# Ewenwan/ORB_SLAM2_SSD_Semantic

Hardware: AMD Instinct MI355X
Metric: ORB extract+match frames/sec on 640x480 TUM RGB-D; bit-exact kp/desc (higher is better)
Workload: dtype u8

## Files before the change

### orb_slam2_ssd_semantic_amd/csrc/orbfe_match.hip

```cpp
#include <stddef.h>
#include <algorithm>
#include <new>

#include <vector>

#include "orbfe_common.h"
#include "orbfe_kernels.h"
#include "orbfe_matcher.h"
#include "orbfe_match_dev.h"

#define BM_WAVES 4
#define BM_QUERIES(Q) (BM_WAVES * (Q) * 32)
#define BM_NEG (-(1 << 30))
#define BM_MAX_NT (1 << 22)

typedef int bm_v4i __attribute__((ext_vector_type(4)));
typedef int bm_v16i __attribute__((ext_vector_type(16)));

__device__ __forceinline__ uint2 bm_expand_byte(uint32_t v, uint32_t mag)
{
    uint32_t lo = 0, hi = 0;
#pragma unroll
    for (int b = 0; b < 4; ++b) {
        lo |= (((v >> b) & 1u) ? mag : (0x100u - mag)) << (8 * b);
        hi |= (((v >> (4 + b)) & 1u) ? mag : (0x100u - mag)) << (8 * b);
    }
    return make_uint2(lo, hi);
}

template <int BM_Q>
__global__ __launch_bounds__(BM_WAVES * 64, 2) void k_match_bf(const uint8_t *__restrict__ q_base,
                                                               const uint8_t *__restrict__ t_base,
                                                               const int32_t *__restrict__ n_arr,
                                                               const int32_t *__restrict__ tn_arr,
                                                               const int32_t *__restrict__ qframe,
                                                               const int32_t *__restrict__ tframe, int cap, int nq_s,
                                                               int nt_s, float nnratio, int th,
                                                               int32_t *__restrict__ match, int32_t *__restrict__ best_o,
                                                               int32_t *__restrict__ second_o)
{
    __shared__ uint2 s_tabq[256], s_tabt[256];
    __shared__ __attribute__((aligned(16))) uint8_t s_tile[2][32 * 256];
    const int pair = blockIdx.y;
    const uint8_t *q = q_base, *t = t_base;
    int nq = nq_s, nt = nt_s;
    int64_t out0 = 0;
    if (n_arr) {
        const int qf = qframe[pair], tf = tframe[pair];
        q = q_base + (int64_t)qf * cap * 32;
        t = t_base + (int64_t)tf * cap * 32;
        nq = min(n_arr[qf], cap);
        nt = min(tn_arr[tf], cap);
        out0 = (int64_t)pair * cap;
    }
    const int tid = threadIdx.x, lane = tid & 63;
    const int wid = __builtin_amdgcn_readfirstlane(tid >> 6);
    constexpr int BM_QW = BM_QUERIES(BM_Q);
    const int q0 = blockIdx.x * BM_QW;
    const int nslots = n_arr ? cap : nq;
    if (q0 >= nslots) return;
    if (q0 >= nq) {
        for (int i = q0 + tid; i < min(q0 + BM_QW, nslots); i += BM_WAVES * 64) {
            match[out0 + i] = -1;
            if (best_o) best_o[out0 + i] = 256;
            if (second_o) second_o[out0 + i] = 256;
        }
        return;
    }
    s_tabq[tid] = bm_expand_byte((uint32_t)tid, 1u);
    s_tabt[tid] = bm_expand_byte((uint32_t)tid, 64u);
    __syncthreads();

    const int c = lane & 31, h = lane >> 5;
    bm_v4i B[BM_Q][8];
#pragma unroll
    for (int u = 0; u < BM_Q; ++u) {
        const int qi = q0 + (wid * BM_Q + u) * 32 + c;
        const uint4 raw = *(const uint4 *)(q + (int64_t)min(qi, nq - 1) * 32 + h * 16);
        const uint32_t rw[4] = {raw.x, raw.y, raw.z, raw.w};
#pragma unroll
        for (int sstep = 0; sstep < 8; ++sstep) {
            const uint32_t b0 = (rw[sstep >> 1] >> (16 * (sstep & 1))) & 0xFFu;
            const uint32_t b1 = (rw[sstep >> 1] >> (16 * (sstep & 1) + 8)) & 0xFFu;
            const uint2 e0 = s_tabq[b0], e1 = s_tabq[b1];
            B[u][sstep] = bm_v4i{(int)e0.x, (int)e0.y, (int)e1.x, (int)e1.y};
        }
    }
    int kb[BM_Q], ks[BM_Q], bi[BM_Q];
#pragma unroll
    for (int u = 0; u < BM_Q; ++u) {
        kb[u] = ks[u] = BM_NEG;
        bi[u] = -1;
    }
    if (nt > 0) {
        const int sr = tid & 31, sw = tid >> 5;
        const uint32_t *t32 = (const uint32_t *)t;
        auto stage_load = [&](int T) -> uint32_t { return t32[(uint32_t)(min(T + sr, nt - 1) * 8 + sw)]; };
        auto stage_store = [&](uint32_t dw, int buf) {
#pragma unroll
            for (int i = 0; i < 4; ++i) {
                const int beta = 4 * sw + i, hh = beta >> 4, bp = beta & 15;
                const int off = (((bp >> 1) * 2 + hh) * 32 + sr) * 16 + (bp & 1) * 8;
                *(uint2 *)(s_tile[buf] + off) = s_tabt[(dw >> (8 * i)) & 0xFFu];
            }
        };
        auto load_a = [&](bm_v4i (&A)[8], int buf) {
#pragma unroll
            for (int sstep = 0; sstep < 8; ++sstep)
                A[sstep] = *(const bm_v4i *)(s_tile[buf] + ((sstep * 2 + h) * 32 + c) * 16);
        };
        bm_v16i cfull;
#pragma unroll
        for (int reg = 0; reg < 16; ++reg) cfull[reg] = 32 - ((reg & 3) + 8 * (reg >> 2) + 4 * h);
        auto chain = [&](const bm_v4i (&A)[8], const bm_v4i (&Bu)[8]) -> bm_v16i {
            bm_v16i acc = cfull;
#pragma unroll
            for (int sstep = 0; sstep < 8; ++sstep) acc = __builtin_amdgcn_mfma_i32_32x32x32_i8(A[sstep], Bu[sstep], acc, 0, 0, 0);
            return acc;
        };
        auto interleave = [&]() {
#pragma unroll
            for (int g = 0; g < 8; ++g) {
                __builtin_amdgcn_sched_group_barrier(0x008, 1, 0);
                __builtin_amdgcn_sched_group_barrier(0x002, 5, 0);
            }
            __builtin_amdgcn_sched_barrier(0);
        };
        auto rank = [&](const bm_v16i &acc, int u, int T, bool mask_tail) {
            int hi[8], lo[8];
#pragma unroll
            for (int p = 0; p < 8; ++p) {
                int k0 = acc[2 * p], k1 = acc[2 * p + 1];
                if (mask_tail) {
                    if (T + ((2 * p) & 3) + 8 * ((2 * p) >> 2) + 4 * h >= nt) k0 = BM_NEG;
                    if (T + ((2 * p + 1) & 3) + 8 * ((2 * p + 1) >> 2) + 4 * h >= nt) k1 = BM_NEG;
                }
                hi[p] = max(k0, k1);
                lo[p] = min(k0, k1);
            }
#pragma unroll
            for (int w = 4; w >= 1; w >>= 1)
#pragma unroll
                for (int p = 0; p < w; ++p) {
                    const int h2 = max(hi[p], hi[p + w]);
                    lo[p] = max(min(hi[p], hi[p + w]), max(lo[p], lo[p + w]));
                    hi[p] = h2;
                }
            const int bprev = kb[u] | 127, sprev = ks[u] | 127;
            const int b = max(bprev, hi[0]);
            const int s2 = max(min(bprev, hi[0]), max(sprev, lo[0]));
            if (b != bprev) bi[u] = T + 32 - (b & 127);
            kb[u] = b;
            ks[u] = s2;
        };

        stage_store(stage_load(0), 0);
        uint32_t g1 = stage_load(32);
        __syncthreads();
        bm_v4i A[8];
        load_a(A, 0);
        bm_v16i acc = chain(A, B[0]);
        int buf = 0, T = 0;
        for (; T + 32 < nt; T += 32) {
            const uint32_t g2 = stage_load(T + 64);
            stage_store(g1, buf ^ 1);
            g1 = g2;
#pragma unroll
            for (int u = 0; u < BM_Q; ++u) {
                bm_v16i nacc;
                if (u + 1 < BM_Q) {
                    nacc = chain(A, B[u + 1]);
                } else {
                    __syncthreads();
                    buf ^= 1;
                    load_a(A, buf);
                    nacc = chain(A, B[0]);
                }
                rank(acc, u, T, false);
                interleave();
                acc = nacc;
            }
        }
#pragma unroll
        for (int u = 0; u < BM_Q; ++u) {
            bm_v16i nacc = acc;
            if (u + 1 < BM_Q) nacc = chain(A, B[u + 1]);
            rank(acc, u, T, true);
            acc = nacc;
        }
    }
#pragma unroll
    for (int u = 0; u < BM_Q; ++u) {
        const int ob = __shfl_xor(kb[u], 32, 64), os = __shfl_xor(ks[u], 32, 64), oi = __shfl_xor(bi[u], 32, 64);
        const int mb = kb[u] >> 7, mo = ob >> 7;
        const bool take_o = mo > mb || (mo == mb && oi >= 0 && (bi[u] < 0 || oi < bi[u]));
        const int m1 = take_o ? mo : mb, idx = take_o ? oi : bi[u];
        const int m2 = max(min(mb, mo), max(ks[u] >> 7, os >> 7));
        const int qi = q0 + (wid * BM_Q + u) * 32 + c;
        if (h == 0 && qi < nslots) {
            const int best = idx >= 0 ? 128 - m1 : 256;
            const int second = m2 > (BM_NEG >> 8) ? 128 - m2 : 256;
            const bool valid = qi < nq;
            int m = -1;
            if (valid && idx >= 0 && best < 256 && best <= th && (float)best < __fmul_rn(nnratio, (float)second)) m = idx;
            match[out0 + qi] = m;
            if (best_o) best_o[out0 + qi] = valid ? best : 256;
            if (second_o) second_o[out0 + qi] = valid ? second : 256;
        }
    }
}

#define BP_TILE 128
__global__ __launch_bounds__(256) void k_match_popc(const uint8_t *__restrict__ q_base, const uint8_t *__restrict__ t_base,
                                                    const int32_t *__restrict__ n_arr, const int32_t *__restrict__ tn_arr,
                                                    const int32_t *__restrict__ qframe,
                                                    const int32_t *__restrict__ tframe, int cap, int nq_s, int nt_s,
                                                    float nnratio, int th, int32_t *__restrict__ match,
                                                    int32_t *__restrict__ best_o, int32_t *__restrict__ second_o)
{
    __shared__ uint4 s_t[BP_TILE][2];
    const int pair = blockIdx.y;
    const uint8_t *q = q_base, *t = t_base;
    int nq = nq_s, nt = nt_s;
    int64_t out0 = 0;
    if (n_arr) {
        const int qf = qframe[pair], tf = tframe[pair];
        q = q_base + (int64_t)qf * cap * 32;
        t = t_base + (int64_t)tf * cap * 32;
        nq = min(n_arr[qf], cap);
        nt = min(tn_arr[tf], cap);
        out0 = (int64_t)pair * cap;
    }
    const int tid = threadIdx.x;
    const int qi = blockIdx.x * 256 + tid;
    const int nslots = n_arr ? cap : nq;
    if ((int)blockIdx.x * 256 >= nslots) return;
    uint32_t qw[8];
    {
        const uint4 *pq = (const uint4 *)(q + (int64_t)min(qi, max(nq - 1, 0)) * 32);
        const uint4 a = nq > 0 ? pq[0] : make_uint4(0, 0, 0, 0), b = nq > 0 ? pq[1] : make_uint4(0, 0, 0, 0);
        qw[0] = a.x; qw[1] = a.y; qw[2] = a.z; qw[3] = a.w; qw[4] = b.x; qw[5] = b.y; qw[6] = b.z; qw[7] = b.w;
    }
    uint32_t k1 = 0xFFFFFFFFu, k2 = 0xFFFFFFFFu;
    for (int T = 0; T < nt; T += BP_TILE) {
        __syncthreads();
        {
            const int r = tid >> 1, hf = tid & 1;
            s_t[r][hf] = ((const uint4 *)(t + (int64_t)min(T + r, nt - 1) * 32))[hf];
        }
        __syncthreads();
        const int rows = min(BP_TILE, nt - T);
        for (int r = 0; r < rows; ++r) {
            const uint4 a = s_t[r][0], b = s_t[r][1];
            uint32_t d = __popc(qw[0] ^ a.x);
            d += __popc(qw[1] ^ a.y);
            d += __popc(qw[2] ^ a.z);
            d += __popc(qw[3] ^ a.w);
            d += __popc(qw[4] ^ b.x);
            d += __popc(qw[5] ^ b.y);
            d += __popc(qw[6] ^ b.z);
            d += __popc(qw[7] ^ b.w);
            const uint32_t k = (d << 22) | (uint32_t)(T + r);
            k2 = min(k2, max(k1, k));
            k1 = min(k1, k);
        }
    }
    if (qi < nslots) {
        const bool valid = qi < nq;
        const int best = k1 != 0xFFFFFFFFu ? (int)(k1 >> 22) : 256;
        const int second = k2 != 0xFFFFFFFFu ? (int)(k2 >> 22) : 256;
        const int idx = k1 != 0xFFFFFFFFu ? (int)(k1 & 0x3FFFFFu) : -1;
        int m = -1;
        if (valid && idx >= 0 && best < 256 && best <= th && (float)best < __fmul_rn(nnratio, (float)second)) m = idx;
        match[out0 + qi] = m;
        if (best_o) best_o[out0 + qi] = valid ? best : 256;
        if (second_o) second_o[out0 + qi] = valid ? second : 256;
    }
}

__global__ __launch_bounds__(256) void k_rot_prune(int32_t *__restrict__ match, const float *__restrict__ a_ang,
                                                   const float *__restrict__ b_ang, int ang_stride,
                                                   const int32_t *__restrict__ n_arr,
                                                   const int32_t *__restrict__ aframe,
                                                   const int32_t *__restrict__ bframe, int cap, int n_s,
                                                   int check_ori, int32_t *__restrict__ nmatches)
{
    __shared__ int s_hist[ORBFE_HISTO_LENGTH];
    __shared__ int s_keep[3];
    __shared__ int s_count;
    const int pair = blockIdx.x, tid = threadIdx.x;
    int n = n_s;
    int32_t *mt = match;
    const float *aa = a_ang, *ba = b_ang;
    if (n_arr) {
        const int af = aframe[pair], bf = bframe[pair];
        n = min(n_arr[af], cap);
        mt = match + (int64_t)pair * cap;
        aa = a_ang + (int64_t)af * cap * ang_stride;
        ba = b_ang + (int64_t)bf * cap * ang_stride;
    }
    if (tid < ORBFE_HISTO_LENGTH) s_hist[tid] = 0;
    if (tid == 0) s_count = 0;
    __syncthreads();
    if (check_ori) {
        for (int i = tid; i < n; i += 256) {
            const int j = mt[i];
            if (j >= 0) atomicAdd(&s_hist[rot_bin(aa[(int64_t)i * ang_stride], ba[(int64_t)j * ang_stride])], 1);
        }
        __syncthreads();
        if (tid == 0) {
            int max1 = 0, max2 = 0, max3 = 0, i1 = -1, i2 = -1, i3 = -1;
            for (int i = 0; i < ORBFE_HISTO_LENGTH; ++i) {
                const int s = s_hist[i];
                if (s > max1) {
                    max3 = max2; max2 = max1; max1 = s;
                    i3 = i2; i2 = i1; i1 = i;
                } else if (s > max2) {
                    max3 = max2; max2 = s;
                    i3 = i2; i2 = i;
                } else if (s > max3) {
                    max3 = s; i3 = i;
                }
            }
            if ((float)max2 < __fmul_rn(0.1f, (float)max1)) { i2 = -1; i3 = -1; }
            else if ((float)max3 < __fmul_rn(0.1f, (float)max1)) { i3 = -1; }
            s_keep[0] = i1; s_keep[1] = i2; s_keep[2] = i3;
        }
        __syncthreads();
    }
    int local = 0;
    for (int i = tid; i < n; i += 256) {
        const int j = mt[i];
        if (j < 0) continue;
        if (check_ori) {
            const int bin = rot_bin(aa[(int64_t)i * ang_stride], ba[(int64_t)j * ang_stride]);
            if (bin != s_keep[0] && bin != s_keep[1] && bin != s_keep[2]) {
                mt[i] = -1;
                continue;
            }
        }
        ++local;
    }
    atomicAdd(&s_count, local);
    __syncthreads();
    if (tid == 0) nmatches[pair] = s_count;
}

__global__ __launch_bounds__(256) void k_hamming_csr(const uint8_t *__restrict__ q, int nq,
                                                     const uint8_t *__restrict__ t, const uint32_t *__restrict__ off,
                                                     const uint32_t *__restrict__ cand, int32_t *__restrict__ best_idx,
                                                     int32_t *__restrict__ best, int32_t *__restrict__ second,
                                                     int32_t *__restrict__ second_idx)
{
    const int i = blockIdx.x * 256 + threadIdx.x;
    if (i >= nq) return;
    Desc8 dq;
    const uint32_t *p = (const uint32_t *)(q + (int64_t)i * 32);
#pragma unroll
    for (int k = 0; k < 8; ++k) dq.w[k] = p[k];
    int b1 = 256, b2 = 256, bi = -1, si = -1;
    for (uint32_t j = off[i]; j < off[i + 1]; ++j) {
        const uint32_t c = cand[j];
        const int d = hamming8(dq, (const uint32_t *)(t + (int64_t)c * 32));
        if (d < b1) { b2 = b1; si = bi; b1 = d; bi = (int)c; }
        else if (d < b2) { b2 = d; si = (int)c; }
    }
    best_idx[i] = bi;
    best[i] = b1;
    second[i] = b2;
    if (second_idx) second_idx[i] = si;
}

__global__ __launch_bounds__(256) void k_hamming_csr_all(const uint8_t *__restrict__ q, int nq, const uint8_t *__restrict__ t,
                                                         const uint32_t *__restrict__ off, const uint32_t *__restrict__ cand,
                                                         uint16_t *__restrict__ dist)
{
    const int i = blockIdx.x * 4 + (threadIdx.x >> 6);
    if (i >= nq) return;
    const int lane = threadIdx.x & 63;
    Desc8 dq;
    const uint32_t *p = (const uint32_t *)(q + (int64_t)i * 32);
#pragma unroll
    for (int k = 0; k < 8; ++k) dq.w[k] = p[k];
    const uint32_t e = off[i + 1];
    for (uint32_t j = off[i] + (uint32_t)lane; j < e; j += 64u)
        dist[j] = (uint16_t)hamming8(dq, (const uint32_t *)(t + (int64_t)cand[j] * 32));
}

extern "C" int32_t orbfe_hamming(const uint8_t a[32], const uint8_t b[32])
{
    int d = 0;
    for (int i = 0; i < 8; ++i) {
        uint32_t x, y;
        memcpy(&x, a + 4 * i, 4);
        memcpy(&y, b + 4 * i, 4);
        d += __builtin_popcount(x ^ y);
    }
    return d;
}

static orbfe_status matcher_create_impl(int32_t device, hipStream_t borrowed, bool borrow, orbfe_matcher **out);
extern "C" orbfe_status orbfe_matcher_create(int32_t device, orbfe_matcher **out) { return matcher_create_impl(device, nullptr, false, out); }
orbfe_status orbfe_internal_matcher_create_on_stream(int32_t device, void *st, orbfe_matcher **out)
{
    return matcher_create_impl(device, (hipStream_t)st, true, out);
}

static orbfe_status matcher_create_impl(int32_t device, hipStream_t borrowed, bool borrow, orbfe_matcher **out)
{
    if (!out) return ORBFE_ERR_ARG;
    *out = nullptr;
    const orbfe_status rs = orb_resolve_device(&device);
    if (rs != ORBFE_OK) return rs;
    orbfe_matcher *m = new (std::nothrow) orbfe_matcher();
    if (!m) return ORBFE_ERR_NOMEM;
    m->device = device;
    DeviceGuard g(device);
    m->own_stream = !borrow;
    if (borrow) m->stream = borrowed;
    if ((!borrow && hipStreamCreateWithFlags(&m->stream, hipStreamNonBlocking) != hipSuccess) ||
        hipEventCreateWithFlags(&m->ev_scratch, hipEventDisableTiming) != hipSuccess) {
        orbfe_set_error("hipStreamCreate / hipEventCreate failed");
        if (m->stream && m->own_stream) (void)hipStreamDestroy(m->stream);
        delete m;
        return ORBFE_ERR_HIP;
    }
    *out = m;
    return ORBFE_OK;
}

extern "C" void *orbfe_matcher_get_stream(orbfe_matcher *m) { return m ? (void *)m->stream : nullptr; }

extern "C" orbfe_status orbfe_matcher_set_bf_kernel(orbfe_matcher *m, int32_t kernel)
{
    if (!m || kernel < 0 || kernel > 1) return ORBFE_ERR_ARG;
    m->bf_kernel = kernel;
    return ORBFE_OK;
}

extern "C" orbfe_status orbfe_internal_matcher_set_bf_tiles(orbfe_matcher *m, int32_t tiles)
{
    if (!m || !orb_match_tiles_ok(tiles)) return ORBFE_ERR_ARG;
    m->bf_tiles = tiles;
    return ORBFE_OK;
}

extern "C" orbfe_status orbfe_matcher_set_projection_kernel(orbfe_matcher *m, int32_t kernel)
{
    if (!m || kernel < 0 || kernel > 1) return ORBFE_ERR_ARG;
    m->proj_fused = kernel == 0;
    return ORBFE_OK;
}

extern "C" void orbfe_matcher_destroy(orbfe_matcher *m)
{
    if (!m) return;
    DeviceGuard g(m->device);
    if (m->stream) (void)hipStreamSynchronize(m->stream);
    if (m->scratch_used) (void)hipEventSynchronize(m->ev_scratch);
    for (auto &b : m->b) b.release();
    m->proj_done.release();
    m->pin_in.release();
    m->pin_out.release();
    if (m->ev_scratch) (void)hipEventDestroy(m->ev_scratch);
    if (m->stream && m->own_stream) (void)hipStreamDestroy(m->stream);
    delete m;
}

template <typename... Args>
static void launch_match_bf(int tiles, int nslots, int npairs, hipStream_t st, Args... args)
{
    const dim3 block(BM_WAVES * 64);
    auto grid = [&](int qw) { return dim3((nslots + qw - 1) / qw, npairs); };
    if (tiles == 1) hipLaunchKernelGGL(k_match_bf<1>, grid(BM_QUERIES(1)), block, 0, st, args...);
    else if (tiles == 2) hipLaunchKernelGGL(k_match_bf<2>, grid(BM_QUERIES(2)), block, 0, st, args...);
    else hipLaunchKernelGGL(k_match_bf<4>, grid(BM_QUERIES(4)), block, 0, st, args...);
}

static orbfe_status launch_bf(int kernel, int tiles, const uint8_t *d_q, int nq, const uint8_t *d_t, int nt, const float *d_qa,
                              const float *d_ta, int ang_stride, float nnratio, int th, int check_ori,
                              int32_t *d_match, int32_t *d_best, int32_t *d_second, int32_t *d_nm, hipStream_t st)
{
    if (nq > 0) {
        if (kernel == 1)
            hipLaunchKernelGGL(k_match_popc, dim3((nq + 255) / 256, 1), dim3(256), 0, st, d_q, d_t, (const int32_t *)nullptr,
                               (const int32_t *)nullptr, (const int32_t *)nullptr, (const int32_t *)nullptr, 0, nq, nt, nnratio, th,
                               d_match, d_best, d_second);
        else
            launch_match_bf(tiles, nq, 1, st, d_q, d_t, (const int32_t *)nullptr, (const int32_t *)nullptr, (const int32_t *)nullptr,
                            (const int32_t *)nullptr, 0, nq, nt, nnratio, th, d_match, d_best, d_second);
        ORBFE_HIP(hipGetLastError());
    }
    const int ori = (check_ori && d_qa && d_ta) ? 1 : 0;
    hipLaunchKernelGGL(k_rot_prune, dim3(1), dim3(256), 0, st, d_match, d_qa, d_ta, ang_stride,
                       (const int32_t *)nullptr, (const int32_t *)nullptr, (const int32_t *)nullptr, 0, nq, ori, d_nm);
    ORBFE_HIP(hipGetLastError());
    return ORBFE_OK;
}

extern "C" orbfe_status orbfe_match_bf_device(orbfe_matcher *m, const uint8_t *d_q, int32_t nq, const uint8_t *d_t,
                                              int32_t nt, const float *d_q_angle, const float *d_t_angle,
                                              float nnratio, int32_t th, int32_t check_ori, int32_t *d_match_q2t,
                                              int32_t *d_best, int32_t *d_second, int32_t *d_nmatches, void *stream)
{
    if (!m || nq < 0 || nt < 0 || nt > BM_MAX_NT || !d_match_q2t || !d_nmatches || (nq > 0 && !d_q) || (nt > 0 && !d_t)) {
        orbfe_set_error("bad argument to orbfe_match_bf_device (train set limited to %d descriptors)", BM_MAX_NT);
        return ORBFE_ERR_ARG;
    }
    DeviceGuard g(m->device);
    return launch_bf(m->bf_kernel, m->bf_tiles, d_q, nq, d_t, nt, d_q_angle, d_t_angle, 1, nnratio, th, check_ori, d_match_q2t, d_best, d_second,
                     d_nmatches, (hipStream_t)stream);
}

extern "C" orbfe_status orbfe_match_bf(orbfe_matcher *m, const uint8_t *q, int32_t nq, const uint8_t *t, int32_t nt,
                                       const float *q_angle, const float *t_angle, float nnratio, int32_t th,
                                       int32_t check_ori, int32_t *match_q2t, int32_t *best, int32_t *second,
                                       int32_t *nmatches)
{
    if (!m || nq < 0 || nt < 0 || nt > BM_MAX_NT || (nq > 0 && (!q || !match_q2t)) || (nt > 0 && !t)) {
        orbfe_set_error("bad argument to orbfe_match_bf (train set limited to %d descriptors)", BM_MAX_NT);
        return ORBFE_ERR_ARG;
    }
    if (nq == 0) {
        if (nmatches) *nmatches = 0;
        return ORBFE_OK;
    }
    DeviceGuard g(m->device);
    hipStream_t st = m->stream;
    ORBFE_HIP(scratch_acquire(m, st));
    const bool ori = check_ori && q_angle && t_angle;
    ORBFE_HIP(m->b[0].ensure((size_t)nq * 32));
    ORBFE_HIP(m->b[1].ensure((size_t)nt * 32));
    ORBFE_HIP(m->b[2].ensure((size_t)nq * 4));
    ORBFE_HIP(m->b[3].ensure((size_t)nt * 4));
    ORBFE_HIP(m->b[4].ensure((size_t)nq * 4));
    ORBFE_HIP(m->b[5].ensure((size_t)nq * 4));
    ORBFE_HIP(m->b[6].ensure((size_t)nq * 4));
    ORBFE_HIP(m->b[7].ensure(4));
    ORBFE_HIP(hipMemcpyAsync(m->b[0].p, q, (size_t)nq * 32, hipMemcpyHostToDevice, st));
    if (nt > 0) ORBFE_HIP(hipMemcpyAsync(m->b[1].p, t, (size_t)nt * 32, hipMemcpyHostToDevice, st));
    if (ori) {
        ORBFE_HIP(hipMemcpyAsync(m->b[2].p, q_angle, (size_t)nq * 4, hipMemcpyHostToDevice, st));
        if (nt > 0) ORBFE_HIP(hipMemcpyAsync(m->b[3].p, t_angle, (size_t)nt * 4, hipMemcpyHostToDevice, st));
    }
    orbfe_status s = launch_bf(m->bf_kernel, m->bf_tiles, m->b[0].as<const uint8_t>(), nq, m->b[1].as<const uint8_t>(), nt,
                               ori ? m->b[2].as<const float>() : nullptr, ori ? m->b[3].as<const float>() : nullptr, 1,
                               nnratio, th, ori ? 1 : 0, m->b[4].as<int32_t>(), m->b[5].as<int32_t>(),
                               m->b[6].as<int32_t>(), m->b[7].as<int32_t>(), st);
    if (s != ORBFE_OK) return s;
    int32_t nm = 0;
    ORBFE_HIP(hipMemcpyAsync(match_q2t, m->b[4].p, (size_t)nq * 4, hipMemcpyDeviceToHost, st));
    if (best) ORBFE_HIP(hipMemcpyAsync(best, m->b[5].p, (size_t)nq * 4, hipMemcpyDeviceToHost, st));
    if (second) ORBFE_HIP(hipMemcpyAsync(second, m->b[6].p, (size_t)nq * 4, hipMemcpyDeviceToHost, st));
    ORBFE_HIP(hipMemcpyAsync(&nm, m->b[7].p, 4, hipMemcpyDeviceToHost, st));
    ORBFE_HIP(hipStreamSynchronize(st));
    if (nmatches) *nmatches = nm;
    return ORBFE_OK;
}

extern "C" orbfe_status orbfe_match_bf_blocks_device(orbfe_matcher *m, const orbfe_keypoint *d_qkps, const uint8_t *d_qdesc,
                                                     const int32_t *d_qn, const orbfe_keypoint *d_tkps, const uint8_t *d_tdesc,
                                                     const int32_t *d_tn, int32_t cap, const int32_t *d_qframe,
                                                     const int32_t *d_tframe, int32_t npairs, float nnratio, int32_t th,
                                                     int32_t check_ori, int32_t *d_match_q2t, int32_t *d_nmatches, void *stream)
{
    return orbfe_internal_match_bf_blocks_tiles(m, d_qkps, d_qdesc, d_qn, d_tkps, d_tdesc, d_tn, cap, d_qframe, d_tframe, npairs, nnratio, th,
                                                check_ori, d_match_q2t, d_nmatches, m ? m->bf_tiles : 0, stream);
}

orbfe_status orbfe_internal_match_bf_blocks_tiles(orbfe_matcher *m, const orbfe_keypoint *d_qkps, const uint8_t *d_qdesc,
                                                  const int32_t *d_qn, const orbfe_keypoint *d_tkps, const uint8_t *d_tdesc,
                                                  const int32_t *d_tn, int32_t cap, const int32_t *d_qframe, const int32_t *d_tframe,
                                                  int32_t npairs, float nnratio, int32_t th, int32_t check_ori, int32_t *d_match_q2t,
                                                  int32_t *d_nmatches, int32_t tiles, void *stream)
{
    if (!m || !d_qkps || !d_qdesc || !d_qn || !d_tkps || !d_tdesc || !d_tn || !d_qframe || !d_tframe || !d_match_q2t ||
        !d_nmatches || cap < 1 || cap > BM_MAX_NT || npairs < 0 || !orb_match_tiles_ok(tiles)) {
        orbfe_set_error("bad argument to orbfe_match_bf_blocks_device / _frames_device (cap 1..%d)", BM_MAX_NT);
        return ORBFE_ERR_ARG;
    }
    if (npairs == 0) return ORBFE_OK;
    DeviceGuard g(m->device);
    hipStream_t st = (hipStream_t)stream;
    if (m->bf_kernel == 1)
        hipLaunchKernelGGL(k_match_popc, dim3((cap + 255) / 256, npairs), dim3(256), 0, st, d_qdesc, d_tdesc, d_qn, d_tn, d_qframe,
                           d_tframe, cap, 0, 0, nnratio, th, d_match_q2t, (int32_t *)nullptr, (int32_t *)nullptr);
    else
        launch_match_bf(tiles, cap, npairs, st, d_qdesc, d_tdesc, d_qn, d_tn, d_qframe, d_tframe, cap, 0, 0, nnratio, th, d_match_q2t,
                        (int32_t *)nullptr, (int32_t *)nullptr);
    ORBFE_HIP(hipGetLastError());
    hipLaunchKernelGGL(k_rot_prune, dim3(npairs), dim3(256), 0, st, d_match_q2t, &d_qkps->angle, &d_tkps->angle, 7, d_qn, d_qframe,
                       d_tframe, cap, 0, check_ori ? 1 : 0, d_nmatches);
    ORBFE_HIP(hipGetLastError());
    return ORBFE_OK;
}

extern "C" orbfe_status orbfe_match_bf_frames_device(orbfe_matcher *m, const orbfe_keypoint *d_kps,
                                                     const uint8_t *d_desc, const int32_t *d_n, int32_t cap,
                                                     const int32_t *d_qframe, const int32_t *d_tframe, int32_t npairs,
                                                     float nnratio, int32_t th, int32_t check_ori,
                                                     int32_t *d_match_q2t, int32_t *d_nmatches, void *stream)
{
    return orbfe_match_bf_blocks_device(m, d_kps, d_desc, d_n, d_kps, d_desc, d_n, cap, d_qframe, d_tframe, npairs, nnratio, th,
                                        check_ori, d_match_q2t, d_nmatches, stream);
}

extern "C" orbfe_status orbfe_hamming_csr_ex(orbfe_matcher *m, const uint8_t *q, int32_t nq, const uint8_t *t, int32_t nt,
                                             const uint32_t *off, const uint32_t *cand, int32_t *best_idx, int32_t *best,
                                             int32_t *second, int32_t *second_idx)
{
    if (!m || nq < 0 || nt < 0 || (nq > 0 && (!q || !off || !best_idx || !best || !second))) {
        orbfe_set_error("bad argument to orbfe_hamming_csr");
        return ORBFE_ERR_ARG;
    }
    if (nq == 0) return ORBFE_OK;
    const size_t nc = off[nq];
    for (int i = 0; i < nq; ++i)
        if (off[i + 1] < off[i]) { orbfe_set_error("CSR offsets must not decrease"); return ORBFE_ERR_ARG; }
    for (size_t k = 0; k < nc; ++k)
        if (cand[k] >= (uint32_t)nt) { orbfe_set_error("candidate index out of range"); return ORBFE_ERR_ARG; }
    DeviceGuard g(m->device);
    hipStream_t st = m->stream;
    ORBFE_HIP(scratch_acquire(m, st));
    ORBFE_HIP(m->b[0].ensure((size_t)nq * 32));
    ORBFE_HIP(m->b[1].ensure((size_t)nt * 32));
    ORBFE_HIP(m->b[2].ensure((size_t)(nq + 1) * 4));
    ORBFE_HIP(m->b[3].ensure(nc * 4));
    ORBFE_HIP(m->b[4].ensure((size_t)nq * 4));
    ORBFE_HIP(m->b[5].ensure((size_t)nq * 4));
    ORBFE_HIP(m->b[6].ensure((size_t)nq * 4));
    ORBFE_HIP(m->b[7].ensure((size_t)nq * 4));
    ORBFE_HIP(hipMemcpyAsync(m->b[0].p, q, (size_t)nq * 32, hipMemcpyHostToDevice, st));
    if (nt > 0) ORBFE_HIP(hipMemcpyAsync(m->b[1].p, t, (size_t)nt * 32, hipMemcpyHostToDevice, st));
    ORBFE_HIP(hipMemcpyAsync(m->b[2].p, off, (size_t)(nq + 1) * 4, hipMemcpyHostToDevice, st));
    if (nc > 0) ORBFE_HIP(hipMemcpyAsync(m->b[3].p, cand, nc * 4, hipMemcpyHostToDevice, st));
    hipLaunchKernelGGL(k_hamming_csr, dim3((nq + 255) / 256), dim3(256), 0, st, m->b[0].as<const uint8_t>(), nq,
                       m->b[1].as<const uint8_t>(), m->b[2].as<const uint32_t>(), m->b[3].as<const uint32_t>(),
                       m->b[4].as<int32_t>(), m->b[5].as<int32_t>(), m->b[6].as<int32_t>(), m->b[7].as<int32_t>());
    ORBFE_HIP(hipGetLastError());
    if (second_idx) ORBFE_HIP(hipMemcpyAsync(second_idx, m->b[7].p, (size_t)nq * 4, hipMemcpyDeviceToHost, st));
    ORBFE_HIP(hipMemcpyAsync(best_idx, m->b[4].p, (size_t)nq * 4, hipMemcpyDeviceToHost, st));
    ORBFE_HIP(hipMemcpyAsync(best, m->b[5].p, (size_t)nq * 4, hipMemcpyDeviceToHost, st));
    ORBFE_HIP(hipMemcpyAsync(second, m->b[6].p, (size_t)nq * 4, hipMemcpyDeviceToHost, st));
    ORBFE_HIP(hipStreamSynchronize(st));
    return ORBFE_OK;
}

extern "C" orbfe_status orbfe_hamming_csr_all(orbfe_matcher *m, const uint8_t *q, int32_t nq, const uint8_t *t, int32_t nt,
                                              const uint32_t *off, const uint32_t *cand, uint16_t *dist)
{
    if (!m || nq < 0 || nt < 0 || (nq > 0 && (!q || !off))) {
        orbfe_set_error("bad argument to orbfe_hamming_csr_all");
        return ORBFE_ERR_ARG;
    }
    if (nq == 0) return ORBFE_OK;
    const size_t nc = off[nq];
    for (int i = 0; i < nq; ++i)
        if (off[i + 1] < off[i]) { orbfe_set_error("CSR offsets must not decrease"); return ORBFE_ERR_ARG; }
    if (nc == 0) return ORBFE_OK;
    if (!cand || !dist || !t) { orbfe_set_error("bad argument to orbfe_hamming_csr_all"); return ORBFE_ERR_ARG; }
    for (size_t k = 0; k < nc; ++k)
        if (cand[k] >= (uint32_t)nt) { orbfe_set_error("candidate index out of range"); return ORBFE_ERR_ARG; }
    DeviceGuard g(m->device);
    hipStream_t st = m->stream;
    ORBFE_HIP(scratch_acquire(m, st));
    ORBFE_HIP(m->b[0].ensure((size_t)nq * 32));
    ORBFE_HIP(m->b[1].ensure((size_t)nt * 32));
    ORBFE_HIP(m->b[2].ensure((size_t)(nq + 1) * 4));
    ORBFE_HIP(m->b[3].ensure(nc * 4));
    ORBFE_HIP(m->b[4].ensure(nc * 2));
    ORBFE_HIP(hipMemcpyAsync(m->b[0].p, q, (size_t)nq * 32, hipMemcpyHostToDevice, st));
    ORBFE_HIP(hipMemcpyAsync(m->b[1].p, t, (size_t)nt * 32, hipMemcpyHostToDevice, st));
    ORBFE_HIP(hipMemcpyAsync(m->b[2].p, off, (size_t)(nq + 1) * 4, hipMemcpyHostToDevice, st));
    ORBFE_HIP(hipMemcpyAsync(m->b[3].p, cand, nc * 4, hipMemcpyHostToDevice, st));
    hipLaunchKernelGGL(k_hamming_csr_all, dim3((nq + 3) / 4), dim3(256), 0, st, m->b[0].as<const uint8_t>(), nq,
                       m->b[1].as<const uint8_t>(), m->b[2].as<const uint32_t>(), m->b[3].as<const uint32_t>(), m->b[4].as<uint16_t>());
    ORBFE_HIP(hipGetLastError());
    ORBFE_HIP(hipMemcpyAsync(dist, m->b[4].p, nc * 2, hipMemcpyDeviceToHost, st));
    ORBFE_HIP(hipStreamSynchronize(st));
    return ORBFE_OK;
}

extern "C" orbfe_status orbfe_hamming_csr(orbfe_matcher *m, const uint8_t *q, int32_t nq, const uint8_t *t, int32_t nt,
                                          const uint32_t *off, const uint32_t *cand, int32_t *best_idx, int32_t *best,
                                          int32_t *second)
{
    return orbfe_hamming_csr_ex(m, q, nq, t, nt, off, cand, best_idx, best, second, nullptr);
}

extern "C" orbfe_status orbfe_hamming_csr_device(orbfe_matcher *m, const uint8_t *d_q, int32_t nq, const uint8_t *d_t,
                                                 const uint32_t *d_off, const uint32_t *d_cand, int32_t *d_best_idx,
                                                 int32_t *d_best, int32_t *d_second, int32_t *d_second_idx, void *stream)
{
    if (!m || nq < 0 || (nq > 0 && (!d_q || !d_t || !d_off || !d_cand || !d_best_idx || !d_best || !d_second))) {
        orbfe_set_error("bad argument to orbfe_hamming_csr_device");
        return ORBFE_ERR_ARG;
    }
    if (nq == 0) return ORBFE_OK;
    DeviceGuard g(m->device);
    hipLaunchKernelGGL(k_hamming_csr, dim3((nq + 255) / 256), dim3(256), 0, (hipStream_t)stream, d_q, nq, d_t, d_off, d_cand,
                       d_best_idx, d_best, d_second, d_second_idx);
    ORBFE_HIP(hipGetLastError());
    return ORBFE_OK;
}
```

### orb_slam2_ssd_semantic_amd/csrc/orbfe_match_dev.h

```cpp
#pragma once

#include "orbfe_common.h"

#define GRID_NC (ORBFE_GRID_COLS * ORBFE_GRID_ROWS)

struct Desc8 {
    uint32_t w[8];
};

__device__ __forceinline__ int hamming8(const Desc8 &a, const uint32_t *__restrict__ b)
{
    int d = 0;
#pragma unroll
    for (int i = 0; i < 8; ++i) d += __popc(a.w[i] ^ b[i]);
    return d;
}

struct Best2 {
    int best, second, idx;
};

__device__ __forceinline__ Best2 merge_best2(const Best2 &lo, const Best2 &hi)
{
    Best2 r;
    if (hi.best < lo.best) {
        r.best = hi.best;
        r.idx = hi.idx;
        r.second = min(lo.best, hi.second);
    } else {
        r.best = lo.best;
        r.idx = lo.idx;
        r.second = min(lo.second, hi.best);
    }
    return r;
}

__device__ __forceinline__ int rot_bin(float a1, float a2)
{
    const float factor = 1.0f / ORBFE_HISTO_LENGTH;
    float rot = __fsub_rn(a1, a2);
    if (rot < 0.0f) rot = __fadd_rn(rot, 360.0f);
    int bin = (int)roundf(__fmul_rn(rot, factor));
    if (bin == ORBFE_HISTO_LENGTH) bin = 0;
    return bin;
}
```

### orb_slam2_ssd_semantic_amd/csrc/orbfe_pipe_plan.h

```cpp
#pragma once

#include <errno.h>
#include <stdint.h>
#include <stdlib.h>

#define ORBFE_PIPE_MAX_PIPES 64
#define ORBFE_PIPE_DEFAULT_QUEUES 4
#define ORBFE_PIPE_MAX_QUEUES 32
#define ORBFE_PIPE_COPY_STREAMS 2

struct OrbPipePlan {
    int32_t P, Q, copies;
    int32_t S;
    int32_t P_eff;
    int32_t side;
    int32_t first, side_index , nstreams;
    int32_t stream_of_pipe[ORBFE_PIPE_MAX_PIPES];
};

static inline int32_t orb_pipe_parse_queues(const char *text)
{
    if (!text || !*text) return ORBFE_PIPE_DEFAULT_QUEUES;
    char *end = nullptr;
    errno = 0;
    const long long v = strtoll(text, &end, 10);
    if (end == text) return ORBFE_PIPE_DEFAULT_QUEUES;
    while (*end == ' ' || *end == '\t' || *end == '\n' || *end == '\r') ++end;
    if (*end) return ORBFE_PIPE_DEFAULT_QUEUES;
    if (errno == ERANGE) return v > 0 ? ORBFE_PIPE_MAX_QUEUES : ORBFE_PIPE_DEFAULT_QUEUES;
    if (v < 1) return ORBFE_PIPE_DEFAULT_QUEUES;
    return v > ORBFE_PIPE_MAX_QUEUES ? ORBFE_PIPE_MAX_QUEUES : (int32_t)v;
}

static inline int32_t orb_pipe_env_queues()
{
    static const int32_t q = orb_pipe_parse_queues(getenv("GPU_MAX_HW_QUEUES"));
    return q;
}

static inline bool orb_pipe_plan(int32_t P, int32_t Q, bool copies, OrbPipePlan *out)
{
    if (!out || P < 1 || P > ORBFE_PIPE_MAX_PIPES) return false;
    OrbPipePlan pl;
    pl.P = P;
    pl.Q = Q < 1 ? 1 : (Q > ORBFE_PIPE_MAX_QUEUES ? ORBFE_PIPE_MAX_QUEUES : Q);
    pl.copies = copies ? 1 : 0;
    pl.first = copies ? ORBFE_PIPE_COPY_STREAMS : 0;
    const int32_t left = pl.Q - pl.first < 1 ? 1 : pl.Q - pl.first;
    pl.side = left >= 2 ? 1 : 0;
    pl.S = left >= P + 1 ? P : (pl.side ? left - 1 : 1);
    pl.P_eff = P < pl.S ? P : pl.S;
    pl.side_index = pl.side ? pl.first + pl.S : -1;
    pl.nstreams = pl.first + pl.S + pl.side;
    for (int32_t i = 0; i < ORBFE_PIPE_MAX_PIPES; ++i) pl.stream_of_pipe[i] = i < P ? i % pl.S : -1;
    *out = pl;
    return true;
}

#ifndef ORBFE_PIPE_LANE_SETS
#define ORBFE_PIPE_LANE_SETS 8
#endif
#define ORBFE_PIPE_LANE_PLACE 1
#ifndef ORBFE_PIPE_LANE_PLACE_AUTO
#define ORBFE_PIPE_LANE_PLACE_AUTO 2
#endif
#ifndef ORBFE_PIPE_LANE_MATCH_TILES
#define ORBFE_PIPE_LANE_MATCH_TILES 2
#endif
#define ORBFE_PIPE_LANE_PLACES 3
#define ORBFE_PIPE_LANES_AUTO 1
#define ORBFE_PIPE_LANE_STREAMS 3

struct OrbPipeLanes {
    int32_t lanes;
    int32_t sets;
};

static inline OrbPipeLanes orb_pipe_lanes(const OrbPipePlan &plan, int32_t nsub, int32_t want_sets = 0)
{
    OrbPipeLanes r;
    r.lanes = (plan.copies == 0 && plan.S < plan.P && plan.S == ORBFE_PIPE_LANE_STREAMS && plan.side == 1 && nsub >= 2) ? 1 : 0;
    const int32_t n = want_sets < 1 ? ORBFE_PIPE_LANE_SETS : want_sets;
    r.sets = r.lanes ? (plan.P < n ? plan.P : n) : plan.P_eff;
    return r;
}
```

Baseline: 341,700.

## Compute brute-force Hamming matching with FP4 scaled MFMA and float-bit rank keys

Replaces the int8 32x32x32 MFMA Hamming-distance chain with the MI355X scaled f8f6f4 MFMA in FP4 mode. Each descriptor bit is encoded as a 4-bit value, so the tile staging, LDS footprint and the number of MFMAs per 32x32 block are all halved. The fp32 accumulator bit pattern is used directly as an integer rank key encoding distance and row, with a compile-time static_assert checking that the ordering is exact. It also raises the match-tile count knob in the pipeline plan from 2 to 4, which adds risk around exactness and scheduling.

```diff
diff --git a/orb_slam2_ssd_semantic_amd/csrc/orbfe_match.hip b/orb_slam2_ssd_semantic_amd/csrc/orbfe_match.hip
--- a/orb_slam2_ssd_semantic_amd/csrc/orbfe_match.hip
+++ b/orb_slam2_ssd_semantic_amd/csrc/orbfe_match.hip
@@ -11,21 +11,25 @@
 
 #define BM_WAVES 4
 #define BM_QUERIES(Q) (BM_WAVES * (Q) * 32)
-#define BM_NEG (-(1 << 30))
 #define BM_MAX_NT (1 << 22)
 
 typedef int bm_v4i __attribute__((ext_vector_type(4)));
 typedef int bm_v16i __attribute__((ext_vector_type(16)));
-
-__device__ __forceinline__ uint2 bm_expand_byte(uint32_t v, uint32_t mag)
-{
-    uint32_t lo = 0, hi = 0;
-#pragma unroll
-    for (int b = 0; b < 4; ++b) {
-        lo |= (((v >> b) & 1u) ? mag : (0x100u - mag)) << (8 * b);
-        hi |= (((v >> (4 + b)) & 1u) ? mag : (0x100u - mag)) << (8 * b);
-    }
-    return make_uint2(lo, hi);
+typedef float bm_v16f __attribute__((ext_vector_type(16)));
+
+__device__ __forceinline__ uint32_t bm_expand_byte(uint32_t v)
+{
+    uint32_t e = 0;
+#pragma unroll
+    for (int b = 0; b < 8; ++b) e |= (((v >> b) & 1u) ? BM_FP4_POS : BM_FP4_NEG) << (4 * b);
+    return e;
+}
+
+__device__ __forceinline__ bm_v16f bm_mfma_fp4(const bm_v4i &a, const bm_v4i &b, const bm_v16f &acc)
+{
+    return __builtin_amdgcn_mfma_scale_f32_32x32x64_f8f6f4(__builtin_shufflevector(a, a, 0, 1, 2, 3, -1, -1, -1, -1),
+                                                           __builtin_shufflevector(b, b, 0, 1, 2, 3, -1, -1, -1, -1), acc, 4, 4, 0,
+                                                           (int)BM_SCALE_TRAIN, 0, (int)BM_SCALE_QUERY);
 }
 
 template <int BM_Q>
@@ -39,8 +43,8 @@
                                                                int32_t *__restrict__ match, int32_t *__restrict__ best_o,
                                                                int32_t *__restrict__ second_o)
 {
-    __shared__ uint2 s_tabq[256], s_tabt[256];
-    __shared__ __attribute__((aligned(16))) uint8_t s_tile[2][32 * 256];
+    __shared__ uint32_t s_tab[256];
+    __shared__ __attribute__((aligned(16))) uint8_t s_tile[2][32 * 128];
     const int pair = blockIdx.y;
     const uint8_t *q = q_base, *t = t_base;
     int nq = nq_s, nt = nt_s;
@@ -67,29 +71,25 @@
         }
         return;
     }
-    s_tabq[tid] = bm_expand_byte((uint32_t)tid, 1u);
-    s_tabt[tid] = bm_expand_byte((uint32_t)tid, 64u);
+    s_tab[tid] = bm_expand_byte((uint32_t)tid);
     __syncthreads();
 
     const int c = lane & 31, h = lane >> 5;
-    bm_v4i B[BM_Q][8];
+    bm_v4i B[BM_Q][4];
 #pragma unroll
     for (int u = 0; u < BM_Q; ++u) {
         const int qi = q0 + (wid * BM_Q + u) * 32 + c;
         const uint4 raw = *(const uint4 *)(q + (int64_t)min(qi, nq - 1) * 32 + h * 16);
         const uint32_t rw[4] = {raw.x, raw.y, raw.z, raw.w};
 #pragma unroll
-        for (int sstep = 0; sstep < 8; ++sstep) {
-            const uint32_t b0 = (rw[sstep >> 1] >> (16 * (sstep & 1))) & 0xFFu;
-            const uint32_t b1 = (rw[sstep >> 1] >> (16 * (sstep & 1) + 8)) & 0xFFu;
-            const uint2 e0 = s_tabq[b0], e1 = s_tabq[b1];
-            B[u][sstep] = bm_v4i{(int)e0.x, (int)e0.y, (int)e1.x, (int)e1.y};
-        }
+        for (int sstep = 0; sstep < 4; ++sstep)
+            B[u][sstep] = bm_v4i{(int)s_tab[rw[sstep] & 0xFFu], (int)s_tab[(rw[sstep] >> 8) & 0xFFu],
+                                 (int)s_tab[(rw[sstep] >> 16) & 0xFFu], (int)s_tab[rw[sstep] >> 24]};
     }
     int kb[BM_Q], ks[BM_Q], bi[BM_Q];
 #pragma unroll
     for (int u = 0; u < BM_Q; ++u) {
-        kb[u] = ks[u] = BM_NEG;
+        kb[u] = ks[u] = BM_KEY_NONE;
         bi[u] = -1;
     }
     if (nt > 0) {
@@ -97,32 +97,28 @@
         const uint32_t *t32 = (const uint32_t *)t;
         auto stage_load = [&](int T) -> uint32_t { return t32[(uint32_t)(min(T + sr, nt - 1) * 8 + sw)]; };
         auto stage_store = [&](uint32_t dw, int buf) {
-#pragma unroll
-            for (int i = 0; i < 4; ++i) {
-                const int beta = 4 * sw + i, hh = beta >> 4, bp = beta & 15;
-                const int off = (((bp >> 1) * 2 + hh) * 32 + sr) * 16 + (bp & 1) * 8;
-                *(uint2 *)(s_tile[buf] + off) = s_tabt[(dw >> (8 * i)) & 0xFFu];
-            }
+            const int off = (((sw & 3) * 2 + (sw >> 2)) * 32 + sr) * 16;
+            *(uint4 *)(s_tile[buf] + off) = make_uint4(s_tab[dw & 0xFFu], s_tab[(dw >> 8) & 0xFFu], s_tab[(dw >> 16) & 0xFFu], s_tab[dw >> 24]);
         };
-        auto load_a = [&](bm_v4i (&A)[8], int buf) {
-#pragma unroll
-            for (int sstep = 0; sstep < 8; ++sstep)
+        auto load_a = [&](bm_v4i (&A)[4], int buf) {
+#pragma unroll
+            for (int sstep = 0; sstep < 4; ++sstep)
                 A[sstep] = *(const bm_v4i *)(s_tile[buf] + ((sstep * 2 + h) * 32 + c) * 16);
         };
-        bm_v16i cfull;
-#pragma unroll
-        for (int reg = 0; reg < 16; ++reg) cfull[reg] = 32 - ((reg & 3) + 8 * (reg >> 2) + 4 * h);
-        auto chain = [&](const bm_v4i (&A)[8], const bm_v4i (&Bu)[8]) -> bm_v16i {
-            bm_v16i acc = cfull;
-#pragma unroll
-            for (int sstep = 0; sstep < 8; ++sstep) acc = __builtin_amdgcn_mfma_i32_32x32x32_i8(A[sstep], Bu[sstep], acc, 0, 0, 0);
-            return acc;
+        bm_v16f cfull;
+#pragma unroll
+        for (int reg = 0; reg < 16; ++reg) cfull[reg] = bm_key_start((reg & 3) + 8 * (reg >> 2) + 4 * h);
+        auto chain = [&](const bm_v4i (&A)[4], const bm_v4i (&Bu)[4]) -> bm_v16i {
+            bm_v16f acc = cfull;
+#pragma unroll
+            for (int sstep = 0; sstep < 4; ++sstep) acc = bm_mfma_fp4(A[sstep], Bu[sstep], acc);
+            return __builtin_bit_cast(bm_v16i, acc);
         };
         auto interleave = [&]() {
 #pragma unroll
-            for (int g = 0; g < 8; ++g) {
+            for (int g = 0; g < 4; ++g) {
                 __builtin_amdgcn_sched_group_barrier(0x008, 1, 0);
-                __builtin_amdgcn_sched_group_barrier(0x002, 5, 0);
+                __builtin_amdgcn_sched_group_barrier(0x002, 13, 0);
             }
             __builtin_amdgcn_sched_barrier(0);
         };
@@ -132,8 +128,8 @@
             for (int p = 0; p < 8; ++p) {
                 int k0 = acc[2 * p], k1 = acc[2 * p + 1];
                 if (mask_tail) {
-                    if (T + ((2 * p) & 3) + 8 * ((2 * p) >> 2) + 4 * h >= nt) k0 = BM_NEG;
-                    if (T + ((2 * p + 1) & 3) + 8 * ((2 * p + 1) >> 2) + 4 * h >= nt) k1 = BM_NEG;
+                    if (T + ((2 * p) & 3) + 8 * ((2 * p) >> 2) + 4 * h >= nt) k0 = BM_KEY_NONE;
+                    if (T + ((2 * p + 1) & 3) + 8 * ((2 * p + 1) >> 2) + 4 * h >= nt) k1 = BM_KEY_NONE;
                 }
                 hi[p] = max(k0, k1);
                 lo[p] = min(k0, k1);
@@ -146,10 +142,10 @@
                     lo[p] = max(min(hi[p], hi[p + w]), max(lo[p], lo[p + w]));
                     hi[p] = h2;
                 }
-            const int bprev = kb[u] | 127, sprev = ks[u] | 127;
+            const int bprev = kb[u] | BM_KEY_FORCE, sprev = ks[u] | BM_KEY_FORCE;
             const int b = max(bprev, hi[0]);
             const int s2 = max(min(bprev, hi[0]), max(sprev, lo[0]));
-            if (b != bprev) bi[u] = T + 32 - (b & 127);
+            if (b != bprev) bi[u] = T + bm_key_row(b);
             kb[u] = b;
             ks[u] = s2;
         };
@@ -157,7 +153,7 @@
         stage_store(stage_load(0), 0);
         uint32_t g1 = stage_load(32);
         __syncthreads();
-        bm_v4i A[8];
+        bm_v4i A[4];
         load_a(A, 0);
         bm_v16i acc = chain(A, B[0]);
         int buf = 0, T = 0;
@@ -192,14 +188,14 @@
 #pragma unroll
     for (int u = 0; u < BM_Q; ++u) {
         const int ob = __shfl_xor(kb[u], 32, 64), os = __shfl_xor(ks[u], 32, 64), oi = __shfl_xor(bi[u], 32, 64);
-        const int mb = kb[u] >> 7, mo = ob >> 7;
+        const int mb = bm_key_m(kb[u]), mo = bm_key_m(ob);
         const bool take_o = mo > mb || (mo == mb && oi >= 0 && (bi[u] < 0 || oi < bi[u]));
         const int m1 = take_o ? mo : mb, idx = take_o ? oi : bi[u];
-        const int m2 = max(min(mb, mo), max(ks[u] >> 7, os >> 7));
+        const int m2 = max(min(mb, mo), max(bm_key_m(ks[u]), bm_key_m(os)));
         const int qi = q0 + (wid * BM_Q + u) * 32 + c;
         if (h == 0 && qi < nslots) {
-            const int best = idx >= 0 ? 128 - m1 : 256;
-            const int second = m2 > (BM_NEG >> 8) ? 128 - m2 : 256;
+            const int best = idx >= 0 ? bm_m_dist(m1) : 256;
+            const int second = m2 > 0 ? bm_m_dist(m2) : 256;
             const bool valid = qi < nq;
             int m = -1;
             if (valid && idx >= 0 && best < 256 && best <= th && (float)best < __fmul_rn(nnratio, (float)second)) m = idx;
diff --git a/orb_slam2_ssd_semantic_amd/csrc/orbfe_match_dev.h b/orb_slam2_ssd_semantic_amd/csrc/orbfe_match_dev.h
--- a/orb_slam2_ssd_semantic_amd/csrc/orbfe_match_dev.h
+++ b/orb_slam2_ssd_semantic_amd/csrc/orbfe_match_dev.h
@@ -15,6 +15,50 @@
     for (int i = 0; i < 8; ++i) d += __popc(a.w[i] ^ b[i]);
     return d;
 }
+
+#define BM_FP4_POS 0x2u
+#define BM_FP4_NEG 0xAu
+#define BM_SCALE_TRAIN 0x84848484
+#define BM_SCALE_QUERY 0x7F7F7F7F
+#define BM_KEY_MULT 32
+#define BM_KEY_OFFSET 40960
+#define BM_KEY_BASE 0x47000000
+#define BM_KEY_FORCE (63 << 8)
+#define BM_KEY_NONE 0
+
+__host__ __device__ constexpr int bm_key_value(int d, int row) { return BM_KEY_MULT * (256 - 2 * d) + (32 - row) + BM_KEY_OFFSET; }
+__host__ __device__ constexpr float bm_key_start(int row) { return (float)(32 - row + BM_KEY_OFFSET); }
+__host__ __device__ constexpr int bm_key_pattern(int v) { return BM_KEY_BASE + ((v - 32768) << 8); }
+__host__ __device__ constexpr int bm_key_bits(int d, int row) { return bm_key_pattern(bm_key_value(d, row)); }
+__host__ __device__ constexpr int bm_key_m(int bits) { return bits >> 14; }
+__host__ __device__ constexpr int bm_m_dist(int m) { return (BM_KEY_BASE >> 14) + 256 - m; }
+__host__ __device__ constexpr int bm_key_dist(int bits) { return bm_m_dist(bm_key_m(bits)); }
+__host__ __device__ constexpr int bm_key_row(int bits) { return 32 - ((bits >> 8) & 63); }
+
+__host__ __device__ constexpr bool bm_key_in_binade(int bits) { return bits >= BM_KEY_BASE && bits < BM_KEY_BASE + (1 << 23); }
+__host__ __device__ constexpr bool bm_key_check(int d)
+{
+    for (int row = 0; row < 32; ++row) {
+        const int v = bm_key_value(d, row), k = bm_key_bits(d, row), f = k | BM_KEY_FORCE;
+        if (__builtin_bit_cast(int, (float)v) != k) return false;
+        if (__builtin_bit_cast(int, bm_key_start(row)) != bm_key_pattern(32 - row + BM_KEY_OFFSET)) return false;
+        if (!bm_key_in_binade(k) || !bm_key_in_binade(f)) return false;
+        if (k <= BM_KEY_NONE || k <= (BM_KEY_NONE | BM_KEY_FORCE)) return false;
+        if (bm_key_dist(k) != d || bm_key_row(k) != row || bm_key_dist(f) != d) return false;
+        if (row < 31 && !(k > bm_key_bits(d, row + 1))) return false;
+        if (row == 31 && d < 256 && !(k > bm_key_bits(d + 1, 0))) return false;
+        if (!(f > bm_key_bits(d, 0)) || (f | BM_KEY_FORCE) != f) return false;
+        if (d > 0 && !(f < bm_key_bits(d - 1, 31))) return false;
+    }
+    return true;
+}
+__host__ __device__ constexpr bool bm_key_check_all()
+{
+    for (int d = 0; d <= 256; ++d)
+        if (!bm_key_check(d)) return false;
+    return bm_key_m(BM_KEY_NONE) == 0 && bm_key_m(BM_KEY_NONE | BM_KEY_FORCE) == 0 && bm_key_m(bm_key_bits(256, 31)) > 0;
+}
+static_assert(bm_key_check_all(), "k_match_bf: the fp32 bit patterns of the accumulators do not rank as (distance, row) keys");
 
 struct Best2 {
     int best, second, idx;
diff --git a/orb_slam2_ssd_semantic_amd/csrc/orbfe_pipe_plan.h b/orb_slam2_ssd_semantic_amd/csrc/orbfe_pipe_plan.h
--- a/orb_slam2_ssd_semantic_amd/csrc/orbfe_pipe_plan.h
+++ b/orb_slam2_ssd_semantic_amd/csrc/orbfe_pipe_plan.h
@@ -65,7 +65,7 @@
 #define ORBFE_PIPE_LANE_PLACE_AUTO 2
 #endif
 #ifndef ORBFE_PIPE_LANE_MATCH_TILES
-#define ORBFE_PIPE_LANE_MATCH_TILES 2
+#define ORBFE_PIPE_LANE_MATCH_TILES 4
 #endif
 #define ORBFE_PIPE_LANE_PLACES 3
 #define ORBFE_PIPE_LANES_AUTO 1
```

After: 350,500, median of 6. +2.6%, better.
